# PauloMigAlmeida/MidoriDB

Hardware: AMD Instinct MI355X
Metric: joined rows/sec, 2x10^8-row INT64 INNER JOIN+GROUP BY, 1/2/4/8 MI355X (higher is better)
Workload: dtype int64

## Files before the change

### midoridb_amd/csrc/mdb_dev_leaf_wide.hip

```cpp
#include "mdb_dev_join_internal.h"

__device__ static inline uint4 lw_load_nt(const void *p)
{
	typedef unsigned int u4_nt __attribute__((ext_vector_type(4)));
	const u4_nt v = __builtin_nontemporal_load(reinterpret_cast<const u4_nt *>(p));
	return make_uint4(v.x, v.y, v.z, v.w);
}


template <bool HAS_R, bool R16 = false >
__global__ __launch_bounds__(LW_THREADS) void k_leaf_wide(gc_args a, uint32_t rem, uint32_t shift, uint32_t nsub)
{
	extern __shared__ __attribute__((aligned(16))) uint32_t lw_lds[];
	__shared__ unsigned long long s_red[LW_THREADS / 64];
	__shared__ uint32_t s_scan[32];
	__shared__ uint32_t s_base;
	const uint32_t T = 1u << rem, mask = T - 1u, leaf = blockIdx.x;
	uint32_t *const s_first = lw_lds;
	uint32_t *const s_cl = lw_lds + T;
	uint32_t *const s_cr = lw_lds + T + T / 2;
	for (uint32_t s = threadIdx.x; s < T; s += LW_THREADS)
		s_first[s] = 0xFFFFFFFFu;
	for (uint32_t s = threadIdx.x; s < (HAS_R ? T : T / 2); s += LW_THREADS)
		s_cl[s] = 0u;
// ... 653 lines not shown
			if (a.keyed_cbits && (cmax >> a.keyed_cbits))
				mdb_raise(a.status, 256u);
			if (!a.keyed_cbits && (cmax >> (32 - (a.kbits < 32 ? a.kbits : 31))))
				mdb_raise(a.status, 16u | (a.rec32 ? 512u : 0u));
		}
		const unsigned long long sums = ((unsigned long long)sum_cl << 32) | (NX ? 0u : sum_cr);
		const unsigned long long want = ((unsigned long long)adds << 32) | radds;
		unsigned long long diff = sums - want;
#pragma unroll
		for (int o = 32; o; o >>= 1)
			diff += __shfl_down(diff, o, MDB_WAVE);
		lw12_barrier();
		if (lane == 0)
			s_red[wave] = diff;
		lw12_barrier();
		diff = 0ull;
#pragma unroll
		for (int w = 0; w < LW_THREADS / 64; w++)
			diff += s_red[w];
		if (diff != 0ull || prod_bad) {
			bad = true;
			break;
		}
	}
	if (bad && threadIdx.x == 0)
		mdb_raise(a.status, 1024u);
	joined = lw_block_sum(joined, s_red);
	if (threadIdx.x == 0 && joined)
		atomicAdd(a.joined, joined);
	if (DN) {
		const unsigned long long cl_all = lw_block_sum((unsigned long long)cleared, s_red);
		if (threadIdx.x == 0 && cl_all)
			atomicAdd(&a.dn_cnt[0], (uint32_t)cl_all);
	}
#pragma unroll
	for (int o = 32; o; o >>= 1) {
		const uint32_t other = (uint32_t)__shfl_xor((int)last_first, o, MDB_WAVE);
		last_first = other > last_first ? other : last_first;
	}
	__syncthreads();
	if (lane == 0)
		s_red[wave] = last_first;
	__syncthreads();
	if (threadIdx.x == 0) {
		uint32_t m = 0;
#pragma unroll
		for (int w = 0; w < LW_THREADS / 64; w++)
			m = (uint32_t)s_red[w] > m ? (uint32_t)s_red[w] : m;
		if (m)
			atomicMax(a.status + 9, m);
	}
}

__global__ __launch_bounds__(LW_THREADS, 8 ) void k_leaf_wide4(gc_args a, uint32_t rem, uint32_t shift, uint32_t nsub)
{
	extern __shared__ __attribute__((aligned(16))) uint32_t lw_lds[];
	__shared__ unsigned long long s_red[LW_THREADS / 64];
	__shared__ uint32_t s_red32[LW_THREADS / 64];
	__shared__ uint32_t s_base;
	const uint32_t T = 1u << rem, mask = T - 1u, leaf = blockIdx.x, wave = threadIdx.x >> 6, lane = mdb_lane();
	uint32_t *const s_fc = lw_lds;
	uint32_t *const s_cl = lw_lds + T;
	for (uint32_t s = threadIdx.x; s < T; s += LW_THREADS)
		s_fc[s] = 0x07FFFFFFu;
	for (uint32_t s = threadIdx.x; s < T / 8; s += LW_THREADS)
		s_cl[s] = 0u;
	uint32_t *const s_rg = s_cl + (T / 8 < 16u ? 16u : T / 8);
	if (a.rg_rec)
		for (uint32_t r = threadIdx.x; r < a.rg_n; r += LW_THREADS)
			s_rg[r] = 0u;
	__syncthreads();
	uint32_t rows_r = 0;
	{
		const uint16_t *const hv_r16 = reinterpret_cast<const uint16_t *>(a.hv_r);
		for (uint32_t sub = 0; sub < nsub; sub++) {
			const uint32_t c0 = a.cnt_r[sub * a.nleaves + leaf], c = c0 < a.cap_r ? c0 : a.cap_r;
			const uint16_t *const src = hv_r16 + (size_t)(leaf * nsub + sub) * a.cap_r;
			rows_r += c;
			for (uint32_t j0 = 0; j0 < c; j0 += 8u * LW_THREADS * LW_UNROLL) {
				uint4 v[LW_UNROLL];
#pragma unroll
				for (int u = 0; u < LW_UNROLL; u++) {
					const uint32_t j = j0 + 8u * ((uint32_t)u * LW_THREADS + threadIdx.x);
					v[u] = make_uint4(0u, 0u, 0u, 0u);
					if (j < c)
						v[u] = lw_load_nt(src + j);
				}
#pragma unroll
				for (int u = 0; u < LW_UNROLL; u++) {
					const uint32_t j = j0 + 8u * ((uint32_t)u * LW_THREADS + threadIdx.x);
					const uint32_t w[4] = { v[u].x, v[u].y, v[u].z, v[u].w };
					if (j + 8u <= c) {
#pragma unroll
						for (int k = 0; k < 8; k++)
							atomicAdd(&s_fc[(w[k >> 1] >> (16 * (k & 1))) & mask], 1u << 27);
					} else {
#pragma unroll
						for (int k = 0; k < 8; k++)
							if (j + k < c)
								atomicAdd(&s_fc[(w[k >> 1] >> (16 * (k & 1))) & mask], 1u << 27);
					}
				}
			}
		}
	}
	__syncthreads();
	uint32_t adds = 0;
	for (uint32_t sub = 0; sub < nsub; sub++) {
		const uint32_t c0 = a.cnt_l[sub * a.nleaves + leaf], c = c0 < a.cap_l ? c0 : a.cap_l;
		const uint64_t *const src = a.hv_l + (size_t)(leaf * nsub + sub) * a.cap_l;
		for (uint32_t i0 = 0; i0 < c; i0 += 2u * LW_THREADS * LW_UNROLL) {
			ulonglong2 v[LW_UNROLL];
#pragma unroll
			for (int u = 0; u < LW_UNROLL; u++) {
				const uint32_t i = i0 + 2u * ((uint32_t)u * LW_THREADS + threadIdx.x);
				v[u] = make_ulonglong2(0ull, 0ull);
				if (i < c)
					v[u] = *reinterpret_cast<const ulonglong2 *>(src + i);
			}
#pragma unroll
			for (int u = 0; u < LW_UNROLL; u++) {
				const uint32_t i = i0 + 2u * ((uint32_t)u * LW_THREADS + threadIdx.x);
				const unsigned long long w[2] = { v[u].x, v[u].y };
#pragma unroll
				for (int k = 0; k < 2; k++)
					if (i + k < c) {
						const uint32_t idx = ((uint32_t)(w[k] >> 32) >> shift) & mask, fc = s_fc[idx];
						if (fc >> 27) {
							atomicMin(&s_fc[idx], (fc & 0xF8000000u) | (uint32_t)w[k]);
							atomicAdd(&s_cl[idx >> 3], 1u << ((idx & 7u) * 4u));
							adds++;
						}
					}
			}
		}
	}
	__syncthreads();
	const uint32_t per_wave = T / (LW_THREADS / 64), words_per_wave = per_wave / 8;
	uint32_t mine = 0, sum_cl = 0, sum_cr = 0;
	for (uint32_t wi = lane; wi < words_per_wave; wi += MDB_WAVE) {
		const uint32_t cw = s_cl[wave * words_per_wave + wi];
		mine += (uint32_t)__popc((cw | (cw >> 1) | (cw >> 2) | (cw >> 3)) & 0x11111111u);
		sum_cl += (((cw & 0x0F0F0F0Fu) + ((cw >> 4) & 0x0F0F0F0Fu)) * 0x01010101u) >> 24;
	}
	{
		uint32_t t = mine;
#pragma unroll
		for (int o = 32; o; o >>= 1)
			t += (uint32_t)__shfl_xor((int)t, o, MDB_WAVE);
		if (lane == 0)
			s_red32[wave] = t;
	}
	__syncthreads();
	if (threadIdx.x == 0) {
		uint32_t total = 0;
#pragma unroll
		for (int w = 0; w < LW_THREADS / 64; w++)
			total += s_red32[w];
		uint32_t nb = 0xFFFFFFFFu;
		if (total && a.rg_rec) {
			atomicAdd(a.rec_valid, total);
			nb = 0u;
		} else if (total) {
			nb = atomicAdd(a.rec_count, total);
			if (nb + total > a.rec_cap) {
				mdb_raise(a.status, 8u);
				nb = 0xFFFFFFFFu;
			} else {
				atomicAdd(a.rec_valid, total);
			}
		}
		s_base = nb;
	}
	__syncthreads();
	const uint32_t base = s_base;
	uint32_t run = 0;
	{
		uint32_t t = lane < wave ? s_red32[lane] : 0u;
#pragma unroll
		for (int o = 32; o; o >>= 1)
			t += (uint32_t)__shfl_xor((int)t, o, MDB_WAVE);
		run = base + t;
	}
	const uint32_t nib = (lane & 7u) * 4u, s_begin = wave * per_wave + lane;
	uint32_t cmax = 0, jsum = 0, last_first = 0, clmax = 0;
	if (a.rg_rec && base != 0xFFFFFFFFu) {
		for (uint32_t s0 = 0; s0 < per_wave; s0 += MDB_WAVE) {
// ... 148 lines not shown
```

### midoridb_amd/csrc/mdb_dev_common.h

```cpp
#ifndef MDB_DEV_COMMON_H
#define MDB_DEV_COMMON_H

#include <hip/hip_runtime.h>
#include <stdint.h>
#include <stdio.h>
#include <string.h>
#include <vector>
#include <string>
#include <unordered_map>
#include "mdb_dev.h"

#define MDB_WAVE 64

struct mdb_prof_rec {
	int name_id;
	hipEvent_t start, stop;
};

struct mdb_col_memo {
	const void *nh_kl, *nh_kr;
	uint64_t nh_nl, nh_nr;
	int nh_result;
	int64_t nh_base;
	uint32_t nh_kbits;
// ... 94 lines not shown
	std::vector<std::vector<const void *>> prof_kernels;
	std::vector<mdb_prof_rec> prof_recs;
	std::vector<std::pair<hipEvent_t, hipEvent_t>> prof_pool;
	size_t prof_pool_used;
};

int mdb_set_err(mdb_dev_ctx *ctx, int code, const char *fmt, ...);
extern "C" int mdb_knob_set(const char *name);
extern "C" int mdb_knob_off(const char *name);
extern "C" long long mdb_knob_int(const char *name, long long dflt);
extern "C" int mdb_knob_str(const char *name, char *buf, size_t cap);

struct mdb_plan_scope {
	mdb_dev_ctx *c;
	explicit mdb_plan_scope(mdb_dev_ctx *ctx) : c(ctx)
	{
		if (c && c->pl_depth++ == 0)
			memset(&c->plan, 0, sizeof(c->plan));
	}
	~mdb_plan_scope()
	{
		if (c && --c->pl_depth == 0) {
			c->ct_calls++;
			c->ct_retries += c->plan.retries;
			c->ct_samples += c->plan.samples;
		}
	}
};

static inline void mdb_explain_sampled(mdb_dev_ctx *ctx)
{
	if (ctx->explain_as_sample) {
		ctx->plan.from_stats = 0;
		ctx->plan.samples = 1;
	}
}

void mdb_memo_switch(mdb_dev_ctx *ctx, const void *kl, uint64_t nl, const void *kr, uint64_t nr);

#define MDB_HIP(ctx, call)                                                                         \
	do {                                                                                       \
		hipError_t e__ = (call);                                                           \
		if (e__ != hipSuccess)                                                             \
			return mdb_set_err((ctx), -MIDORIDB_INTERNAL, "%s failed: %s (%s:%d)", #call, \
					   hipGetErrorString(e__), __FILE__, __LINE__);            \
	} while (0)

int mdb_cached_alloc(mdb_dev_ctx *ctx, size_t bytes, void **dptr);
int mdb_cached_free(mdb_dev_ctx *ctx, void *dptr);

int mdb_arena_begin(mdb_dev_ctx *ctx, size_t total_bytes);
void *mdb_arena_take(mdb_dev_ctx *ctx, size_t bytes);
#define MDB_ZERO_BLK_OFF 128u
#define MDB_ZERO_BLK_SLOT 4096u
#define MDB_ZERO_BLK_WORDS (2u * MDB_ZERO_BLK_SLOT + 2048u)
static inline size_t mdb_align_up(size_t x) { return (x + 255) & ~(size_t)255; }

int mdb_aux_begin(mdb_dev_ctx *ctx, hipStream_t *saved_main);
int mdb_aux_end(mdb_dev_ctx *ctx, hipStream_t saved_main);
int mdb_aux_join(mdb_dev_ctx *ctx);

void mdb_prof_begin(mdb_dev_ctx *ctx, const char *name, const void *kernel);
void mdb_prof_end(mdb_dev_ctx *ctx);

#define MDB_LAUNCH(ctx, name, kernel, grid, block, ...)                                            \
	do {                                                                                       \
		mdb_prof_begin((ctx), (name), (const void *)(kernel));                             \
		hipLaunchKernelGGL(kernel, dim3(grid), dim3(block), 0, (ctx)->stream, __VA_ARGS__); \
		mdb_prof_end((ctx));                                                               \
		hipError_t le__ = hipGetLastError();                                               \
		if (le__ != hipSuccess)                                                            \
			return mdb_set_err((ctx), -MIDORIDB_INTERNAL, "launch %s failed: %s", (name), \
					   hipGetErrorString(le__));                               \
	} while (0)

#define MDB_LAUNCH_LDS(ctx, name, kernel, grid, block, lds_bytes, ...)                             \
	do {                                                                                       \
		mdb_prof_begin((ctx), (name), (const void *)(kernel));                             \
		hipLaunchKernelGGL(kernel, dim3(grid), dim3(block), (lds_bytes), (ctx)->stream, __VA_ARGS__); \
		mdb_prof_end((ctx));                                                               \
		hipError_t le__ = hipGetLastError();                                               \
		if (le__ != hipSuccess)                                                            \
			return mdb_set_err((ctx), -MIDORIDB_INTERNAL, "launch %s failed: %s", (name), \
					   hipGetErrorString(le__));                               \
	} while (0)

#ifdef __HIPCC__

__host__ __device__ static inline uint64_t mdb_fmix64(uint64_t k)
{
	k ^= k >> 33;
	k *= 0xff51afd7ed558ccdULL;
	k ^= k >> 33;
	k *= 0xc4ceb9fe1a85ec53ULL;
	k ^= k >> 33;
	return k;
}

__host__ __device__ static inline uint32_t mdb_fmix32(uint32_t h)
{
	h ^= h >> 16;
	h *= 0x85EBCA6Bu;
	h ^= h >> 13;
	h *= 0xC2B2AE35u;
	h ^= h >> 16;
	return h;
// ... 78 lines not shown
```

### midoridb_amd/csrc/mdb_dev_partition.hip

```cpp
#include <stdlib.h>
#include <type_traits>
#include "mdb_dev_internal.h"

#define PART_THREADS 512
#define PART_WAVES (PART_THREADS / MDB_WAVE)
#define PART_ITEMS (MDB_TILE / PART_THREADS)
#define PART_WAVE_SPAN (MDB_TILE / PART_WAVES)
#define PART_MAX_R (1u << MDB_MAX_RADIX_BITS)
#define PART_FEW_DIGITS 4u
#define PART_INVALID 0xFFFFFFFFu

struct mdb_level_args {
	const int64_t *keys;
	const uint64_t *nullbits;
	uint64_t n;
	const uint64_t *hv_in;
	const uint32_t *rid_in;
	const mdb_tile_desc *tiles;
	uint64_t *hv_out;
	uint32_t *rid_out;
	uint32_t *hist;
	uint32_t ntiles;
	uint32_t R;
	uint32_t shift;
	uint32_t mbits;
	uint32_t mode;
	uint32_t inverse_out;
	uint32_t *cursor;
	uint32_t cap;
	uint32_t skip_zero;
	uint32_t nsub;
	uint32_t *status;
	uint32_t narrow;
	int64_t narrow_base;
	uint32_t narrow_kbits;
	uint32_t keys32;
	const uint32_t *filter;
	uint32_t filter_words, filter_shift;
	uint32_t *minmax_out;
	uint32_t *minmax_final;
	const uint32_t *range_in;
	unsigned long long *minmax64_out;
	const long long *range64_in;
	const uint64_t *pay_in[2];
	uint64_t *pay_out[2];
	uint32_t npay;
	uint32_t keep_on;
	int64_t keep_lo, keep_hi;
	uint32_t own_on;
	int64_t own_lo, own_hi;
	uint32_t out16_shift;
	uint32_t fold64;
};

template <bool CF = false, bool RIDW = false>
// ... 1064 lines not shown
		a.keep_on = (flt && l == 0 && flt->keep_on) ? 1u : 0u;
		a.keep_lo = flt ? flt->keep_lo : 0;
		a.keep_hi = flt ? flt->keep_hi : 0;
		a.minmax_out = (flt && l == 0 && flt->minmax_out) ? flt->minmax_tiles : NULL;
		a.minmax_final = a.minmax_out ? flt->minmax_out : NULL;
		a.range_in = (flt && l == 0) ? flt->range_in : NULL;
		a.minmax64_out = (flt && l == 0 && flt->minmax64_out) ? flt->minmax64_tiles : NULL;
		a.range64_in = (flt && l == 0) ? flt->range64_in : NULL;
		a.filter = (flt && l == 1) ? flt->bits : NULL;
		a.filter_words = flt ? flt->words : 0u;
		a.filter_shift = flt ? flt->shift : 0u;
		if (a.mode == MDB_DIGIT_RADIX) {
			const int b = l == 0 ? bits1 : bits2;
			a.shift = (uint32_t)((w32 ? 32 : 64) - used_bits - b);
			a.mbits = (uint32_t)b;
		} else {
			uint32_t mb = 1;
			while ((1u << mb) < R)
				mb++;
			a.shift = 0;
			a.mbits = mb;
		}

		if (fast0 && l == 0) {
			const bool cursor_ext = !dry && flt && flt->cursor0_ext && nreg0 <= flt->cursor0_ext_words;
			uint32_t *cursor0 = cursor_ext ? flt->cursor0_ext : (uint32_t *)cv.take((size_t)nreg0 * 4);
			uint32_t *reg_nt = (uint32_t *)cv.take(((size_t)nreg0 + 1) * 4);
			const uint32_t next_tiles = (uint32_t)(n / MDB_TILE) + nreg0 + 1;
			mdb_tile_desc *next_desc = stop0 ? NULL : (mdb_tile_desc *)cv.take((size_t)next_tiles * sizeof(mdb_tile_desc));
			if (cv.failed)
				return -MIDORIDB_INTERNAL;
			if (!dry) {
				const bool cf = a.narrow && narrow_kbits && !(flags & PART_F_KEYS32) && mode == MDB_DIGIT_RADIX && !raw_hv && !want_rid;
				a.cursor = cursor0;
				a.cap = cap0;
				a.nsub = PART_NSUB;
				a.status = ctx->d_status;
				if (!cursor_ext)
					MDB_HIP(ctx, hipMemsetAsync(cursor0, 0, (size_t)nreg0 * 4, ctx->stream));
				const long long t2min = mdb_knob_int("MDB_TILE2_MIN", 0);
				const bool t2 = n >= (t2min > 0 ? (uint64_t)t2min : (1ull << 25)) &&
						!mdb_knob_off("MDB_TILE2");
				const uint32_t ntiles2 = (uint32_t)((n + (uint64_t)PART_TMUL * MDB_TILE - 1) / ((uint64_t)PART_TMUL * MDB_TILE));
				if (raw_hv && fold32 && t2) {
					a.ntiles = ntiles2;
					MDB_LAUNCH(ctx, "sort_scatter_l0_w32", (k_part_scatter<pf_word_raw_w32_t2>), grid8(ntiles2), PART_THREADS, a);
				} else if (raw_hv && fold32) {
					MDB_LAUNCH(ctx, "sort_scatter_l0_w32", (k_part_scatter<pf_word_raw_w32>), grid8(ntiles), PART_THREADS, a);
				} else if (raw_hv) {
					MDB_LAUNCH(ctx, "sort_scatter_l0", (k_part_scatter<pf_word_raw>), grid8(ntiles), PART_THREADS, a);
				} else if (w32) {
					if (out16) {
						a.out16_shift = 32u - narrow_kbits;
						if (cf && t2) {
							a.ntiles = ntiles2;
							MDB_LAUNCH(ctx, "part_scatter_l0_w32", (k_part_scatter<pf_key_w32_out16_cf_t2>),
								   grid8(ntiles2), PART_THREADS, a);
						} else if (cf) {
							MDB_LAUNCH(ctx, "part_scatter_l0_w32", (k_part_scatter<pf_key_w32_out16_cf>),
								   grid8(ntiles), PART_THREADS, a);
						} else {
							MDB_LAUNCH(ctx, "part_scatter_l0_w32", (k_part_scatter<pf_key_w32_out16>),
								   grid8(ntiles), PART_THREADS, a);
						}
					} else if (cf) {
						MDB_LAUNCH(ctx, "part_scatter_l0_w32", (k_part_scatter<pf_key_w32_cf>),
							   grid8(ntiles), PART_THREADS, a);
					} else {
						MDB_LAUNCH(ctx, "part_scatter_l0_w32", (k_part_scatter<pf_key_w32>), grid8(ntiles), PART_THREADS, a);
					}
					if (a.minmax_out)
						MDB_LAUNCH(ctx, "part_minmax", k_part_minmax_reduce, MM_GROUPS, MM_THREADS, (const uint32_t *)a.minmax_out, a.ntiles, flt->minmax_out);
				} else if (npay) {
					if (!cf || a.narrow != 1u)
						return mdb_set_err(ctx, -MIDORIDB_INTERNAL, "payload cells travel with the compact narrow form's hash | row id words only");
					a.npay = (uint32_t)npay;
					for (int c = 0; c < npay; c++) {
						a.pay_in[c] = reinterpret_cast<const uint64_t *>(flt->pay_in[c]);
						a.pay_out[c] = pay_buf[c];
					}
					MDB_LAUNCH(ctx, "part_scatter_l0_pay", (k_part_scatter<pf_key_cf_pay>), grid8(ntiles), PART_THREADS, a);
				} else if (want_rid && a.range64_in) {
					MDB_LAUNCH(ctx, "part_scatter_l0_rid_pruned", (k_part_scatter<pf_key_rid_r64>), grid8(ntiles), PART_THREADS, a);
				} else if (want_rid) {
					MDB_LAUNCH(ctx, "part_scatter_l0_rid", (k_part_scatter<pf_key_rid>), grid8(ntiles), PART_THREADS, a);
				} else if (a.minmax64_out) {
					MDB_LAUNCH(ctx, "part_scatter_l0", (k_part_scatter<pf_key_mm64>), grid8(ntiles), PART_THREADS, a);
					MDB_LAUNCH(ctx, "part_minmax", k_part_minmax64_reduce, 1, 1024, (const unsigned long long *)a.minmax64_out, ntiles,
						   flt->minmax64_out);
				} else if (a.range_in && cf && t2) {
					a.ntiles = ntiles2;
					MDB_LAUNCH(ctx, "part_scatter_l0_pruned", (k_part_scatter<pf_key_cf_t2>), grid8(ntiles2), PART_THREADS, a);
				} else if (a.range_in && cf) {
					MDB_LAUNCH(ctx, "part_scatter_l0_pruned", (k_part_scatter<pf_key_cf>),
						   grid8(ntiles), PART_THREADS, a);
				} else if (a.range_in) {
					MDB_LAUNCH(ctx, "part_scatter_l0_pruned", (k_part_scatter<pf_key>), grid8(ntiles), PART_THREADS, a);
				} else if (cf && t2) {
					a.ntiles = ntiles2;
					MDB_LAUNCH(ctx, "part_scatter_l0", (k_part_scatter<pf_key_cf_t2>), grid8(ntiles2), PART_THREADS, a);
				} else if (cf) {
					MDB_LAUNCH(ctx, "part_scatter_l0", (k_part_scatter<pf_key_cf>), grid8(ntiles),
						   PART_THREADS, a);
				} else {
					MDB_LAUNCH(ctx, "part_scatter_l0", (k_part_scatter<pf_key>), grid8(ntiles), PART_THREADS, a);
				}
				if (!stop0) {
// ... 372 lines not shown
```

Measured before the change: 178.7 billion.

## Flatten leaf_wide4 sub-region loops into a double-buffered cursor loader

Replaces the per-sub-region nested loops in k_leaf_wide4 with one flattened iteration space. A per-block prefix scan of the sub-region counts is kept in LDS, and a wave-uniform cursor maps chunk indices to addresses. Loads are double-buffered (two register batches of depth 3), so global loads for the next batch are issued while LDS atomics run on the current one. This also removes tail inefficiency on small sub-regions. In exchange it adds a cap of 8 sub-regions with an error raise, extra cursor arithmetic and register pressure, and it drops the barrier between the right and left phases.

```diff
diff --git a/midoridb_amd/csrc/mdb_dev_leaf_wide.hip b/midoridb_amd/csrc/mdb_dev_leaf_wide.hip
--- a/midoridb_amd/csrc/mdb_dev_leaf_wide.hip
+++ b/midoridb_amd/csrc/mdb_dev_leaf_wide.hip
@@ -729,6 +729,52 @@
 	}
 }
 
+#define LW_NSUB 8u
+#define LW4_DEPTH 3
+
+struct lw_cursor {
+	uint32_t j, c0, c1, cnt;
+};
+
+__device__ static inline lw_cursor lw_cursor_begin(const uint32_t *seg)
+{
+	lw_cursor at;
+	at.j = 0u;
+	at.c0 = 0u;
+	at.c1 = (uint32_t)__builtin_amdgcn_readfirstlane((int)seg[LW_NSUB]);
+	at.cnt = (uint32_t)__builtin_amdgcn_readfirstlane((int)seg[0]);
+	return at;
+}
+
+template <uint32_t PER, bool NT, typename W>
+__device__ static inline uint32_t lw_chunk_load(const W *tbl, uint32_t cap, const uint32_t *seg, uint32_t total, lw_cursor &at, uint32_t q, uint4 &v)
+{
+	const uint32_t last = total - 1u, q0 = (uint32_t)__builtin_amdgcn_readfirstlane((int)q);
+	const uint32_t q_lo = q0 < last ? q0 : last, q_hi = q0 + (MDB_WAVE - 1u) < last ? q0 + (MDB_WAVE - 1u) : last, qc = q < last ? q : last;
+	while (q_lo >= at.c1 && at.j + 1u < LW_NSUB) {
+		at.j++;
+		at.c0 = at.c1;
+		at.c1 = (uint32_t)__builtin_amdgcn_readfirstlane((int)seg[LW_NSUB + at.j]);
+		at.cnt = (uint32_t)__builtin_amdgcn_readfirstlane((int)seg[at.j]);
+	}
+	uint32_t first = at.c0, words = at.cnt, skip = 0u;
+	if (q_hi >= at.c1) {
+		uint32_t jj = at.j, c1 = at.c1;
+		while (qc >= c1 && jj + 1u < LW_NSUB) {
+			first = c1;
+			jj++;
+			c1 = seg[LW_NSUB + jj];
+		}
+		words = seg[jj];
+		skip = (jj - at.j) * cap;
+	}
+	const uint32_t word = (qc - first) * PER;
+	const char *const src = reinterpret_cast<const char *>(tbl + (size_t)at.j * cap) + (uint32_t)((skip + word) * (uint32_t)sizeof(W));
+	v = NT ? lw_load_nt(src) : *reinterpret_cast<const uint4 *>(src);
+	const uint32_t nv = words - word < PER ? words - word : PER;
+	return q < total ? nv : 0u;
+}
+
 __global__ __launch_bounds__(LW_THREADS, 8 ) void k_leaf_wide4(gc_args a, uint32_t rem, uint32_t shift, uint32_t nsub)
 {
 	extern __shared__ __attribute__((aligned(16))) uint32_t lw_lds[];
@@ -738,6 +784,16 @@
 	const uint32_t T = 1u << rem, mask = T - 1u, leaf = blockIdx.x, wave = threadIdx.x >> 6, lane = mdb_lane();
 	uint32_t *const s_fc = lw_lds;
 	uint32_t *const s_cl = lw_lds + T;
+	if (nsub > LW_NSUB || (((uint64_t)(a.cap_l > a.cap_r ? a.cap_l : a.cap_r) * (8u * LW_NSUB)) >> 32)) {
+		if (threadIdx.x == 0)
+			mdb_raise(a.status, 4096u);
+		return;
+	}
+	uint32_t *const s_seg = reinterpret_cast<uint32_t *>(s_red);
+	static_assert(4u * LW_NSUB * sizeof(uint32_t) <= sizeof(s_red), "the counts of a digit's sub-regions do not fit s_red");
+	uint32_t seg_cnt = 0;
+	if (threadIdx.x < 2u * LW_NSUB && (threadIdx.x & (LW_NSUB - 1u)) < nsub)
+		seg_cnt = (threadIdx.x < LW_NSUB ? a.cnt_r : a.cnt_l)[(threadIdx.x & (LW_NSUB - 1u)) * a.nleaves + leaf];
 	for (uint32_t s = threadIdx.x; s < T; s += LW_THREADS)
 		s_fc[s] = 0x07FFFFFFu;
 	for (uint32_t s = threadIdx.x; s < T / 8; s += LW_THREADS)
@@ -746,70 +802,101 @@
 	if (a.rg_rec)
 		for (uint32_t r = threadIdx.x; r < a.rg_n; r += LW_THREADS)
 			s_rg[r] = 0u;
+	{
+		const uint32_t seg_cap = threadIdx.x < LW_NSUB ? a.cap_r : a.cap_l;
+		seg_cnt = seg_cnt < seg_cap ? seg_cnt : seg_cap;
+		uint32_t run = threadIdx.x < LW_NSUB ? (seg_cnt + 7u) >> 3 : (seg_cnt + 1u) >> 1;
+#pragma unroll
+		for (uint32_t o = 1; o < LW_NSUB; o <<= 1) {
+			const uint32_t before = (uint32_t)__shfl_up((int)run, o, (int)LW_NSUB);
+			if ((threadIdx.x & (LW_NSUB - 1u)) >= o)
+				run += before;
+		}
+		if (threadIdx.x < 2u * LW_NSUB) {
+			const uint32_t at = (threadIdx.x / LW_NSUB) * 2u * LW_NSUB + (threadIdx.x & (LW_NSUB - 1u));
+			s_seg[at] = seg_cnt;
+			s_seg[at + LW_NSUB] = run;
+		}
+	}
 	__syncthreads();
 	uint32_t rows_r = 0;
-	{
-		const uint16_t *const hv_r16 = reinterpret_cast<const uint16_t *>(a.hv_r);
-		for (uint32_t sub = 0; sub < nsub; sub++) {
-			const uint32_t c0 = a.cnt_r[sub * a.nleaves + leaf], c = c0 < a.cap_r ? c0 : a.cap_r;
-			const uint16_t *const src = hv_r16 + (size_t)(leaf * nsub + sub) * a.cap_r;
-			rows_r += c;
-			for (uint32_t j0 = 0; j0 < c; j0 += 8u * LW_THREADS * LW_UNROLL) {
-				uint4 v[LW_UNROLL];
-#pragma unroll
-				for (int u = 0; u < LW_UNROLL; u++) {
-					const uint32_t j = j0 + 8u * ((uint32_t)u * LW_THREADS + threadIdx.x);
-					v[u] = make_uint4(0u, 0u, 0u, 0u);
-					if (j < c)
-						v[u] = lw_load_nt(src + j);
-				}
-#pragma unroll
-				for (int u = 0; u < LW_UNROLL; u++) {
-					const uint32_t j = j0 + 8u * ((uint32_t)u * LW_THREADS + threadIdx.x);
-					const uint32_t w[4] = { v[u].x, v[u].y, v[u].z, v[u].w };
-					if (j + 8u <= c) {
-#pragma unroll
-						for (int k = 0; k < 8; k++)
+#pragma unroll
+	for (int j = 0; j < (int)LW_NSUB; j++)
+		rows_r += s_seg[j];
+	const uint32_t total_r = (uint32_t)__builtin_amdgcn_readfirstlane((int)s_seg[2u * LW_NSUB - 1u]);
+	const uint32_t total_l = (uint32_t)__builtin_amdgcn_readfirstlane((int)s_seg[4u * LW_NSUB - 1u]);
+	if (total_r) {
+		const uint16_t *const hv_r16 = reinterpret_cast<const uint16_t *>(a.hv_r) + (size_t)leaf * nsub * a.cap_r;
+		lw_cursor at = lw_cursor_begin(s_seg);
+		uint4 va[LW4_DEPTH], vb[LW4_DEPTH];
+		auto issue_r = [&](uint32_t batch, uint4(&v)[LW4_DEPTH]) -> uint32_t {
+			uint32_t nvs = 0;
+#pragma unroll
+			for (int u = 0; u < LW4_DEPTH; u++)
+				nvs |= lw_chunk_load<8u, true>(hv_r16, a.cap_r, s_seg, total_r, at, (batch * LW4_DEPTH + (uint32_t)u) * LW_THREADS + threadIdx.x, v[u]) << (4 * u);
+			return nvs;
+		};
+		auto count_r = [&](const uint4(&v)[LW4_DEPTH], uint32_t nvs) {
+#pragma unroll
+			for (int u = 0; u < LW4_DEPTH; u++) {
+				const uint32_t w[4] = { v[u].x, v[u].y, v[u].z, v[u].w }, nv = (nvs >> (4 * u)) & 15u;
+				if (nv == 8u) {
+#pragma unroll
+					for (int k = 0; k < 8; k++)
+						atomicAdd(&s_fc[(w[k >> 1] >> (16 * (k & 1))) & mask], 1u << 27);
+				} else {
+#pragma unroll
+					for (int k = 0; k < 8; k++)
+						if ((uint32_t)k < nv)
 							atomicAdd(&s_fc[(w[k >> 1] >> (16 * (k & 1))) & mask], 1u << 27);
-					} else {
-#pragma unroll
-						for (int k = 0; k < 8; k++)
-							if (j + k < c)
-								atomicAdd(&s_fc[(w[k >> 1] >> (16 * (k & 1))) & mask], 1u << 27);
-					}
-				}
-			}
-		}
-	}
-	__syncthreads();
+				}
+			}
+		};
+		const uint32_t nbat = (total_r + LW4_DEPTH * LW_THREADS - 1u) / (LW4_DEPTH * LW_THREADS);
+		uint32_t na = issue_r(0u, va), nb;
+		for (uint32_t b = 0; b < nbat; b += 2u) {
+			nb = issue_r(b + 1u, vb);
+			count_r(va, na);
+			na = issue_r(b + 2u, va);
+			count_r(vb, nb);
+		}
+	}
 	uint32_t adds = 0;
-	for (uint32_t sub = 0; sub < nsub; sub++) {
-		const uint32_t c0 = a.cnt_l[sub * a.nleaves + leaf], c = c0 < a.cap_l ? c0 : a.cap_l;
-		const uint64_t *const src = a.hv_l + (size_t)(leaf * nsub + sub) * a.cap_l;
-		for (uint32_t i0 = 0; i0 < c; i0 += 2u * LW_THREADS * LW_UNROLL) {
-			ulonglong2 v[LW_UNROLL];
-#pragma unroll
-			for (int u = 0; u < LW_UNROLL; u++) {
-				const uint32_t i = i0 + 2u * ((uint32_t)u * LW_THREADS + threadIdx.x);
-				v[u] = make_ulonglong2(0ull, 0ull);
-				if (i < c)
-					v[u] = *reinterpret_cast<const ulonglong2 *>(src + i);
-			}
-#pragma unroll
-			for (int u = 0; u < LW_UNROLL; u++) {
-				const uint32_t i = i0 + 2u * ((uint32_t)u * LW_THREADS + threadIdx.x);
-				const unsigned long long w[2] = { v[u].x, v[u].y };
+	if (total_l) {
+		const uint64_t *const hv_l = a.hv_l + (size_t)leaf * nsub * a.cap_l;
+		lw_cursor at = lw_cursor_begin(s_seg + 2u * LW_NSUB);
+		uint4 va[LW4_DEPTH], vb[LW4_DEPTH];
+		auto issue_l = [&](uint32_t batch, uint4(&v)[LW4_DEPTH]) -> uint32_t {
+			uint32_t nvs = 0;
+#pragma unroll
+			for (int u = 0; u < LW4_DEPTH; u++)
+				nvs |= lw_chunk_load<2u, false>(hv_l, a.cap_l, s_seg + 2u * LW_NSUB, total_l, at, (batch * LW4_DEPTH + (uint32_t)u) * LW_THREADS + threadIdx.x, v[u]) << (4 * u);
+			return nvs;
+		};
+		auto count_l = [&](const uint4(&v)[LW4_DEPTH], uint32_t nvs) {
+#pragma unroll
+			for (int u = 0; u < LW4_DEPTH; u++) {
+				const uint32_t w[4] = { v[u].x, v[u].y, v[u].z, v[u].w }, nv = (nvs >> (4 * u)) & 15u;
 #pragma unroll
 				for (int k = 0; k < 2; k++)
-					if (i + k < c) {
-						const uint32_t idx = ((uint32_t)(w[k] >> 32) >> shift) & mask, fc = s_fc[idx];
+					if ((uint32_t)k < nv) {
+						const uint32_t idx = (w[2 * k + 1] >> shift) & mask, fc = s_fc[idx];
 						if (fc >> 27) {
-							atomicMin(&s_fc[idx], (fc & 0xF8000000u) | (uint32_t)w[k]);
+							atomicMin(&s_fc[idx], (fc & 0xF8000000u) | w[2 * k]);
 							atomicAdd(&s_cl[idx >> 3], 1u << ((idx & 7u) * 4u));
 							adds++;
 						}
 					}
 			}
+		};
+		const uint32_t nbat = (total_l + LW4_DEPTH * LW_THREADS - 1u) / (LW4_DEPTH * LW_THREADS);
+		uint32_t na = issue_l(0u, va), nb = issue_l(1u, vb);
+		lw12_barrier();
+		for (uint32_t b = 0; b < nbat; b += 2u) {
+			count_l(va, na);
+			na = issue_l(b + 2u, va);
+			count_l(vb, nb);
+			nb = issue_l(b + 3u, vb);
 		}
 	}
 	__syncthreads();
diff --git a/profiles/leaf_wide4_loader/cmp_dumps.py b/profiles/leaf_wide4_loader/cmp_dumps.py
--- /dev/null
+++ b/profiles/leaf_wide4_loader/cmp_dumps.py
@@ -0,0 +1,17 @@
+import glob
+import os
+import sys
+
+import numpy as np
+
+a, b = sys.argv[1], sys.argv[2]
+fa = sorted(os.path.basename(f) for f in glob.glob(a + "/*.npy"))
+fb = sorted(os.path.basename(f) for f in glob.glob(b + "/*.npy"))
+assert fa and fa == fb, (fa, fb)
+for f in fa:
+    x, y = np.load(os.path.join(a, f)), np.load(os.path.join(b, f))
+    same = x.shape == y.shape and np.array_equal(x, y)
+    print(f, x.shape, "identical" if same else "DIFFERENT")
+    assert same
+    os.remove(os.path.join(a, f))
+    os.remove(os.path.join(b, f))
diff --git a/profiles/leaf_wide4_loader/kstats.py b/profiles/leaf_wide4_loader/kstats.py
--- /dev/null
+++ b/profiles/leaf_wide4_loader/kstats.py
@@ -0,0 +1,16 @@
+import csv
+import glob
+import statistics
+import sys
+
+d, tag = sys.argv[1], sys.argv[2]
+rows = {}
+for f in glob.glob(d + "/**/*kernel_trace.csv", recursive=True):
+    with open(f) as fh:
+        for r in csv.DictReader(fh):
+            rows.setdefault(r["Kernel_Name"], []).append((int(r["End_Timestamp"]) - int(r["Start_Timestamp"])) / 1000.0)
+for k, v in sorted(rows.items(), key=lambda kv: -sum(kv[1])):
+    if sum(v) < 50 and "leaf_wide4" not in k:
+        continue
+    sd = statistics.pstdev(v) if len(v) > 1 else 0.0
+    print(f"{tag} {k.split('(')[0][:60]:60s} n={len(v):3d} avg_us={statistics.mean(v):8.1f} sd_us={sd:6.1f} min_us={min(v):8.1f}")
```

After: 176.6 billion. 0.988x the previous value.

## Add persistent streaming 512-way level-0 scatter kernel with fused min/max reduction

Applied to the files above, without the earlier changes.

Adds a persistent-grid scatter kernel for the 32-bit-key, 16-bit-output level-0 partition. Each workgroup streams over a contiguous row range, using a register ring of nontemporal prefetched loads. It overlaps counting of the next tile with the scattered stores of the previous tile, which are staged in LDS. The separate min/max reduction launch is folded into the kernel using a last-block ticket. This costs more LDS and register pressure, plus a specialised path with tighter eligibility conditions.

```diff
diff --git a/midoridb_amd/csrc/mdb_dev_common.h b/midoridb_amd/csrc/mdb_dev_common.h
--- a/midoridb_amd/csrc/mdb_dev_common.h
+++ b/midoridb_amd/csrc/mdb_dev_common.h
@@ -170,6 +170,7 @@
 int mdb_arena_begin(mdb_dev_ctx *ctx, size_t total_bytes);
 void *mdb_arena_take(mdb_dev_ctx *ctx, size_t bytes);
 #define MDB_ZERO_BLK_OFF 128u
+#define MDB_ST_TICKET 48u
 #define MDB_ZERO_BLK_SLOT 4096u
 #define MDB_ZERO_BLK_WORDS (2u * MDB_ZERO_BLK_SLOT + 2048u)
 static inline size_t mdb_align_up(size_t x) { return (x + 255) & ~(size_t)255; }
diff --git a/midoridb_amd/csrc/mdb_dev_partition.hip b/midoridb_amd/csrc/mdb_dev_partition.hip
--- a/midoridb_amd/csrc/mdb_dev_partition.hip
+++ b/midoridb_amd/csrc/mdb_dev_partition.hip
@@ -1,6 +1,7 @@
 #include <stdlib.h>
 #include <type_traits>
 #include "mdb_dev_internal.h"
+#include "mdb_dev_scatter512.h"
 
 #define PART_THREADS 512
 #define PART_WAVES (PART_THREADS / MDB_WAVE)
@@ -1171,7 +1172,39 @@
 				} else if (w32) {
 					if (out16) {
 						a.out16_shift = 32u - narrow_kbits;
-						if (cf && t2) {
+						const bool stream = cf && t2 && !a.range_in && !a.keep_on && !a.own_on && n >= 1 && n < (1ull << 31) && R <= S512_D &&
+								    (!a.minmax_out || a.minmax_final) && !mdb_knob_off("MDB_STREAM512");
+						if (stream) {
+							s512_args sa;
+							memset(&sa, 0, sizeof(sa));
+							sa.keys = reinterpret_cast<const long long *>(keys);
+							sa.nullbits = reinterpret_cast<const unsigned long long *>(nullbits);
+							sa.n = (uint32_t)n;
+							sa.key_lo = narrow_base;
+							sa.kbits = narrow_kbits;
+							sa.rem = narrow_kbits - (uint32_t)bits1;
+							sa.R = R;
+							sa.out = reinterpret_cast<uint16_t *>(a.hv_out);
+							sa.cursor = cursor0;
+							sa.cap = cap0;
+							sa.nsub = PART_NSUB;
+							sa.status = ctx->d_status;
+							const uint32_t s_tile = S512_THREADS * S512_RPT;
+							const uint32_t s_grid = s512_grid(keys, sa.n, s_tile, S512_WG_PER_CU * (uint32_t)ctx->num_cus, &sa.rows_per_wg);
+							sa.mm_wg = a.minmax_out;
+							sa.mm_ticket = ctx->d_status + MDB_ST_TICKET;
+							sa.mm_final = a.minmax_final;
+							const size_t lds = s512_stream_lds(s_tile);
+							if (sa.mm_wg && nullbits)
+								MDB_LAUNCH_LDS(ctx, "part_scatter_l0_w32", (k_scatter512_stream<S512_THREADS, S512_RPT, true, true>), s_grid, S512_THREADS, lds, sa);
+							else if (sa.mm_wg)
+								MDB_LAUNCH_LDS(ctx, "part_scatter_l0_w32", (k_scatter512_stream<S512_THREADS, S512_RPT, false, true>), s_grid, S512_THREADS, lds, sa);
+							else if (nullbits)
+								MDB_LAUNCH_LDS(ctx, "part_scatter_l0_w32", (k_scatter512_stream<S512_THREADS, S512_RPT, true, false>), s_grid, S512_THREADS, lds, sa);
+							else
+								MDB_LAUNCH_LDS(ctx, "part_scatter_l0_w32", (k_scatter512_stream<S512_THREADS, S512_RPT, false, false>), s_grid, S512_THREADS, lds, sa);
+							a.minmax_out = NULL;
+						} else if (cf && t2) {
 							a.ntiles = ntiles2;
 							MDB_LAUNCH(ctx, "part_scatter_l0_w32", (k_part_scatter<pf_key_w32_out16_cf_t2>),
 								   grid8(ntiles2), PART_THREADS, a);
diff --git a/midoridb_amd/csrc/mdb_dev_scatter512.h b/midoridb_amd/csrc/mdb_dev_scatter512.h
--- /dev/null
+++ b/midoridb_amd/csrc/mdb_dev_scatter512.h
@@ -0,0 +1,311 @@
+#ifndef MDB_DEV_SCATTER512_H
+#define MDB_DEV_SCATTER512_H
+
+#include "mdb_dev_scatter4096.h"
+
+#define S512_D 512u
+#define S512_THREADS 512
+#define S512_RPT 32
+#define S512_RING 8
+#define S512_WG_PER_CU 2u
+
+struct s512_args {
+	const long long *keys;
+	const unsigned long long *nullbits;
+	uint32_t n;
+	long long key_lo;
+	uint32_t kbits, rem;
+	uint32_t R;
+	uint16_t *out;
+	uint32_t *cursor;
+	uint32_t cap, nsub;
+	uint32_t *status;
+	uint32_t rows_per_wg;
+	uint32_t *mm_wg, *mm_ticket, *mm_final;
+};
+
+__device__ static inline uint32_t s512_mixk(uint32_t x, uint32_t s, uint32_t mask)
+{
+	x ^= x >> s;
+	x = (x * 0x85EBCA6Bu) & mask;
+	x ^= x >> s;
+	x = (x * 0xC2B2AE35u) & mask;
+	x ^= x >> s;
+	return x;
+}
+
+template <int THREADS, int RPT , bool NULLS = false, bool MM = true , int RING_ = S512_RING,
+	  int ABLATE = 0 >
+__global__ __launch_bounds__(THREADS, 4 ) void k_scatter512_stream(s512_args a)
+{
+	constexpr uint32_t TILE = THREADS * RPT, D = S512_D, NCHUNK = TILE / 64u, NPAIR = RPT / 2, RING = RING_;
+	constexpr uint32_t WB = 4;
+	static_assert(TILE <= 32768u && THREADS == (int)D && RPT % 4 == 0 && NPAIR % RING == 0 && (TILE / 32u) % 2u == 0, "tile shape");
+	extern __shared__ __attribute__((aligned(16))) uint32_t s512_lds[];
+	uint32_t *const s_cnt = s512_lds;
+	uint32_t *const s_delta = s_cnt + D + 64;
+	uint32_t *const s_chunk = s_delta + D;
+	uint32_t *const s_mark = s_chunk + NCHUNK;
+	uint32_t *const s_tmp = s_mark + TILE / 32u;
+	uint16_t *const s_stage = reinterpret_cast<uint16_t *>(s_tmp + 32);
+	__shared__ uint32_t s_any_bad, s_last;
+
+	const uint32_t lane = mdb_lane(), sub = blockIdx.x % a.nsub, R = a.R;
+	const uint32_t none = R << a.rem;
+	const uint32_t hmask = a.kbits >= 32u ? 0xFFFFFFFFu : ((1u << a.kbits) - 1u), hshift = (a.kbits + 1u) >> 1;
+	const uint64_t limit = (1ull << a.kbits) - 1ull;
+	const uint64_t le = mdb_lanemask_lt() | (1ull << lane);
+	const uint32_t lead = (uint32_t)(reinterpret_cast<uintptr_t>(a.keys) >> 3) & 1u;
+	const long long *const fkeys = a.keys - lead;
+	const uint32_t nf = a.n + lead;
+	for (uint32_t i = threadIdx.x; i < D + 64; i += THREADS)
+		s_cnt[i] = 0u;
+	if (threadIdx.x == 0)
+		s_any_bad = 0u;
+	uint32_t seen_min = 0xFFFFFFFFu, seen_max = 0u;
+
+	const uint32_t r_begin = blockIdx.x * a.rows_per_wg;
+	const uint32_t r_end = r_begin >= nf ? r_begin : (nf - r_begin > a.rows_per_wg ? r_begin + a.rows_per_wg : nf);
+
+	ulonglong2 pre[RING];
+	uint32_t hs[RPT];
+#define S512_REQUEST(P, t0, tlen, tid_)                                                                                  \
+	do {                                                                                                             \
+		if (ABLATE & 2) {                                                                                        \
+			const unsigned long long i_ = (t0) + 2u * ((uint32_t)(P) * THREADS + (tid_));                    \
+			pre[(P) % RING] = make_ulonglong2((unsigned long long)a.key_lo + ((i_ * 0x9E3779B1ull) & limit), \
+							  (unsigned long long)a.key_lo + (((i_ + 1u) * 0x9E3779B1ull) & limit)); \
+		} else {	 \
+			typedef unsigned long long ull2_nt_ __attribute__((ext_vector_type(2)));                         \
+			const uint32_t last_ = ((tlen) - 1u) & ~1u, e0_ = 2u * ((uint32_t)(P) * THREADS + (tid_));      \
+			const ull2_nt_ v_ = __builtin_nontemporal_load(reinterpret_cast<const ull2_nt_ *>(              \
+				reinterpret_cast<const char *>(fkeys + (t0)) + (size_t)(e0_ < last_ ? e0_ : last_) * 8u)); \
+			pre[(P) % RING] = make_ulonglong2(v_.x, v_.y);                                                   \
+		}                                                                                                        \
+	} while (0)
+#define S512_COUNT(r_, t0, tlen, tid_)                                                                                   \
+	do {                                                                                                             \
+		const uint32_t e_ = 2u * ((uint32_t)((r_) >> 1) * THREADS + (tid_)) + (uint32_t)((r_) & 1);             \
+		const unsigned long long kk_ = ((r_) & 1) ? pre[((r_) >> 1) % RING].y : pre[((r_) >> 1) % RING].x;      \
+		bool ok_ = e_ < (tlen) && (t0) + e_ >= lead;                                                             \
+		if (NULLS && ok_) {                                                                                      \
+			const uint32_t row_ = (t0) + e_ - lead;                                                          \
+			ok_ = !((a.nullbits[row_ >> 6] >> (row_ & 63u)) & 1ull);                                         \
+		}                                                                                                        \
+		const unsigned long long rel_ = kk_ - (unsigned long long)a.key_lo;                                      \
+		const bool take_ = ok_ && rel_ <= limit;                                                                 \
+		oow |= ok_ && !take_;                                                                                    \
+		if (MM) {                                                                                                \
+			seen_min = min(seen_min, take_ ? (uint32_t)rel_ : 0xFFFFFFFFu);                                  \
+			seen_max = max(seen_max, take_ ? (uint32_t)rel_ : 0u);                                           \
+		}                                                                                                        \
+		uint32_t h_ = s512_mixk((uint32_t)rel_, hshift, hmask);	 \
+		asm volatile("" : "+v"(h_));                                                                             \
+		h_ = take_ ? h_ : none;                                                                                  \
+		atomicAdd(&s_cnt[h_ >> a.rem], 1u);                                                                      \
+		hs[r_] = h_;                                                                                             \
+	} while (0)
+
+	uint32_t row0 = r_begin, staged_row0 = 0;
+	uint32_t len = (r_end - row0) < TILE ? (r_end - row0) : TILE, staged_total = 0u;
+	if (len) {
+		uint32_t tid = threadIdx.x;
+		asm volatile("" : "+v"(tid));
+#pragma unroll
+		for (int p = 0; p < (int)RING; p++)
+			S512_REQUEST(p, row0, len, tid);
+	}
+	shw_barrier();
+
+	for (;;) {
+		uint32_t tid = threadIdx.x;
+		asm volatile("" : "+v"(tid));
+		const uint32_t wave = tid >> 6;
+		const uint32_t nrow0 = row0 + len;
+		const uint32_t nlen = len ? ((r_end - nrow0) < TILE ? (r_end - nrow0) : TILE) : 0u;
+		const uint32_t prow0 = nlen ? nrow0 : row0;
+		const uint32_t plen = nlen ? nlen : len;
+		bool oow = false;
+
+		if (len) {
+#pragma unroll
+			for (int k = 0; k < RPT; k++) {
+				S512_COUNT(k, row0, len, tid);
+				if (k & 1)
+					__builtin_amdgcn_sched_barrier(0);
+				if ((k & 1) && (k >> 1) + (int)RING < (int)NPAIR)
+					S512_REQUEST((k >> 1) + (int)RING, row0, len, tid);
+				else if (k & 1)
+					S512_REQUEST((k >> 1) + (int)RING - (int)NPAIR, prow0, plen, tid);
+			}
+			if (oow)
+				mdb_raise(a.status, 128u);
+		}
+#pragma unroll
+		for (int k0 = 0; k0 < RPT; k0 += (int)WB) {
+			if ((uint32_t)k0 * THREADS < staged_total) {
+				uint64_t m[WB];
+				uint32_t ord[WB], g[WB];
+				uint16_t sv[WB];
+#pragma unroll
+				for (int u = 0; u < (int)WB; u++) {
+					const uint32_t c = (uint32_t)(k0 + u) * (THREADS / 64) + wave;
+					m[u] = *reinterpret_cast<const uint64_t *>(&s_mark[2u * c]);
+					ord[u] = s_chunk[c];
+					sv[u] = s_stage[(uint32_t)(k0 + u) * THREADS + tid];
+				}
+#pragma unroll
+				for (int u = 0; u < (int)WB; u++) {
+					ord[u] += (uint32_t)__popcll(m[u] & le) - 1u;
+					ord[u] = ord[u] < D ? ord[u] : D - 1u;
+					g[u] = s_delta[ord[u]];
+				}
+#pragma unroll
+				for (int u = 0; u < (int)WB; u++) {
+					const uint32_t i = (uint32_t)(k0 + u) * THREADS + tid;
+					const bool put = i < staged_total;
+					uint32_t gi = i + g[u];
+					if (ABLATE & 16)
+						gi = staged_row0 + i;
+					if (!(ABLATE & 1)) {
+						if (put)
+							a.out[gi] = sv[u];
+					} else if (put && sv[u] == (uint16_t)0xFFF1u && gi == 0xFFFFFFFFu) {
+						a.out[0] = sv[u];
+					}
+				}
+			}
+		}
+		shw_barrier();
+		if (!len)
+			break;
+
+		const uint32_t cnt = tid < R ? s_cnt[tid] : 0u;
+		for (uint32_t i = tid; i < TILE / 32u; i += THREADS)
+			s_mark[i] = 0u;
+		if (tid == 0)
+			s_chunk[0] = 0u;
+		uint32_t tot;
+		const uint32_t ex = shw_block_excl_scan(cnt + (cnt ? 65536u : 0u), s_tmp, THREADS / 64, &tot);
+		const uint32_t tile_total = (uint32_t)__builtin_amdgcn_readfirstlane((int)(tot & 0xFFFFu));
+		const uint32_t start = ex & 0xFFFFu, ord = ex >> 16;
+		uint32_t base = 0u;
+		if (cnt) {
+			base = atomicAdd(&a.cursor[sub * R + tid], cnt);
+			atomicOr(&s_mark[start >> 5], 1u << (start & 31u));
+			for (uint32_t c = (start >> 6) + 1u; (c << 6) <= start + cnt && c < NCHUNK; c++)
+				s_chunk[c] = ord + 1u;
+		}
+		if (tid < R)
+			s_cnt[tid] = start;
+		if (tid == 0)
+			s_cnt[R] = TILE;
+		shw_barrier();
+
+#pragma unroll
+		for (int r = 0; r < RPT; r++) {
+			uint32_t pos = atomicAdd(&s_cnt[hs[r] >> a.rem], 1u);
+			pos = pos < TILE ? pos : TILE;
+			s_stage[pos] = (uint16_t)hs[r];
+		}
+		if (cnt) {
+			if (base + cnt > a.cap) {
+				mdb_raise(a.status, 2u);
+				s_any_bad = 1u;
+			}
+			s_delta[ord] = (tid * a.nsub + sub) * a.cap + base - start;
+		}
+		shw_barrier();
+		s_cnt[tid] = 0u;
+		if (tid == 0)
+			s_cnt[D] = 0u;
+		staged_total = __builtin_amdgcn_readfirstlane((int)s_any_bad) ? 0u : tile_total;
+		staged_row0 = row0;
+		row0 = nrow0;
+		len = nlen;
+		shw_barrier();
+		if (tid == 0)
+			s_any_bad = 0u;
+	}
+#undef S512_REQUEST
+#undef S512_COUNT
+
+	if (MM) {
+		const uint32_t wave = threadIdx.x >> 6;
+#pragma unroll
+		for (int o = MDB_WAVE / 2; o > 0; o >>= 1) {
+			seen_min = min(seen_min, (uint32_t)__shfl_xor((int)seen_min, o, MDB_WAVE));
+			seen_max = max(seen_max, (uint32_t)__shfl_xor((int)seen_max, o, MDB_WAVE));
+		}
+		if (lane == 0) {
+			s_tmp[2u * wave] = seen_min;
+			s_tmp[2u * wave + 1u] = seen_max;
+		}
+		__syncthreads();
+		if (threadIdx.x == 0) {
+			uint32_t mn = 0xFFFFFFFFu, mx = 0u;
+#pragma unroll
+			for (int w = 0; w < THREADS / 64; w++) {
+				mn = min(mn, s_tmp[2 * w]);
+				mx = max(mx, s_tmp[2 * w + 1]);
+			}
+			__hip_atomic_store(&a.mm_wg[2u * blockIdx.x], mn, __ATOMIC_RELAXED, __HIP_MEMORY_SCOPE_AGENT);
+			__hip_atomic_store(&a.mm_wg[2u * blockIdx.x + 1u], mx, __ATOMIC_RELAXED, __HIP_MEMORY_SCOPE_AGENT);
+			__threadfence();
+			s_last = atomicAdd(a.mm_ticket, 1u) == gridDim.x - 1u;
+		}
+		__syncthreads();
+		if (s_last) {
+			__threadfence();
+			uint32_t mn = 0xFFFFFFFFu, mx = 0u;
+			for (uint32_t b = threadIdx.x; b < gridDim.x; b += THREADS) {
+				mn = min(mn, __hip_atomic_load(&a.mm_wg[2u * b], __ATOMIC_RELAXED, __HIP_MEMORY_SCOPE_AGENT));
+				mx = max(mx, __hip_atomic_load(&a.mm_wg[2u * b + 1u], __ATOMIC_RELAXED, __HIP_MEMORY_SCOPE_AGENT));
+			}
+#pragma unroll
+			for (int o = MDB_WAVE / 2; o > 0; o >>= 1) {
+				mn = min(mn, (uint32_t)__shfl_xor((int)mn, o, MDB_WAVE));
+				mx = max(mx, (uint32_t)__shfl_xor((int)mx, o, MDB_WAVE));
+			}
+			if (lane == 0) {
+				s_tmp[2u * wave] = mn;
+				s_tmp[2u * wave + 1u] = mx;
+			}
+			__syncthreads();
+			if (threadIdx.x == 0) {
+				mn = 0xFFFFFFFFu;
+				mx = 0u;
+#pragma unroll
+				for (int w = 0; w < THREADS / 64; w++) {
+					mn = min(mn, s_tmp[2 * w]);
+					mx = max(mx, s_tmp[2 * w + 1]);
+				}
+				a.mm_final[0] = mn;
+				a.mm_final[1] = mx;
+				__hip_atomic_store(a.mm_ticket, 0u, __ATOMIC_RELAXED, __HIP_MEMORY_SCOPE_AGENT);
+			}
+		}
+	}
+}
+
+static inline size_t s512_stream_lds(uint32_t tile)
+{
+	return (size_t)4 * (S512_D + 64 + S512_D + tile / 64 + tile / 32 + 32) + 2 * ((size_t)tile + 64);
+}
+
+static inline uint32_t s512_grid(const void *keys, uint32_t n, uint32_t tile, uint32_t slots, uint32_t *rows_per_wg)
+{
+	const uint64_t nf = (uint64_t)n + ((reinterpret_cast<uintptr_t>(keys) >> 3) & 1u);
+	uint64_t grid = (nf + tile - 1) / tile;
+	if (grid > slots)
+		grid = slots;
+	if (grid < 1)
+		grid = 1;
+	uint64_t rpw = ((nf + grid - 1) / grid + 1) & ~1ull;
+	while (grid > 1 && (grid - 1) * rpw >= nf)
+		grid--;
+	*rows_per_wg = (uint32_t)rpw;
+	return (uint32_t)grid;
+}
+
+#endif
diff --git a/profiles/micro/scatter512_stream.hip b/profiles/micro/scatter512_stream.hip
--- /dev/null
+++ b/profiles/micro/scatter512_stream.hip
@@ -0,0 +1,226 @@
+#include "mdb_dev_partition.hip"
+#include <cstdlib>
+#include <vector>
+#include <algorithm>
+
+#define CK(x) do { hipError_t e_ = (x); if (e_ != hipSuccess) { printf("%s: %s (line %d)\n", #x, hipGetErrorString(e_), __LINE__); exit(1); } } while (0)
+#define NSUB 8u
+#define KBITS 23u
+#define DBITS 9u
+#define KEY_LO 1000ll
+#define MULT 0x9E3779B1ull
+
+__global__ void k_gen(long long *keys, uint32_t n, uint32_t nv)
+{
+	for (uint32_t i = blockIdx.x * blockDim.x + threadIdx.x; i < n; i += gridDim.x * blockDim.x)
+		keys[i] = KEY_LO + (long long)(((unsigned long long)(i % nv) * MULT) % nv);
+}
+
+__global__ void k_expect(const long long *keys, uint32_t n, uint32_t *expect)
+{
+	for (uint32_t i = blockIdx.x * blockDim.x + threadIdx.x; i < n; i += gridDim.x * blockDim.x)
+		atomicAdd(&expect[(uint32_t)(keys[i] - KEY_LO)], 1u);
+}
+
+__global__ void k_walk(const uint16_t *out, const uint32_t *cursor, uint32_t cap, uint32_t *got, unsigned long long *stats )
+{
+	const uint32_t D = 1u << DBITS, rem = KBITS - DBITS, r = blockIdx.x * blockDim.x + threadIdx.x;
+	if (r >= D * NSUB)
+		return;
+	const uint32_t d = r / NSUB, sub = r % NSUB;
+	uint32_t cnt = cursor[sub * D + d];
+	unsigned long long rows = 0, err = 0;
+	if (cnt > cap) {
+		err++;
+		cnt = cap;
+	}
+	const uint16_t *w = out + (size_t)r * cap;
+	for (uint32_t i = 0; i < cnt; i++) {
+		const uint32_t h = (d << rem) | (w[i] & ((1u << rem) - 1u));
+		if ((h & 0xFFFFu) != w[i]) {
+			err++;
+			continue;
+		}
+		atomicAdd(&got[mdb_unmixk(h, KBITS)], 1u);
+		rows++;
+	}
+	atomicAdd(&stats[0], rows);
+	atomicAdd(&stats[1], err);
+}
+
+__global__ void k_compare(const uint32_t *expect, const uint32_t *got, uint32_t nvals, unsigned long long *stats)
+{
+	for (uint32_t i = blockIdx.x * blockDim.x + threadIdx.x; i < nvals; i += gridDim.x * blockDim.x)
+		if (expect[i] != got[i])
+			atomicAdd(&stats[1], 1ull);
+}
+
+struct bufs {
+	long long *keys;
+	unsigned long long *nullbits;
+	uint16_t *out;
+	uint32_t *cursor, *status, *expect, *got, *mm;
+	unsigned long long *stats;
+	uint32_t n, nv, cap;
+};
+
+static void check(bufs &b, bool range)
+{
+	uint32_t st[64];
+	unsigned long long h[2];
+	CK(hipMemset(b.got, 0, (size_t)4 << KBITS));
+	CK(hipMemset(b.stats, 0, 16));
+	hipLaunchKernelGGL(k_walk, dim3((NSUB << DBITS) / 64), dim3(64), 0, 0, b.out, b.cursor, b.cap, b.got, b.stats);
+	hipLaunchKernelGGL(k_compare, dim3(1024), dim3(256), 0, 0, b.expect, b.got, 1u << KBITS, b.stats);
+	CK(hipDeviceSynchronize());
+	CK(hipMemcpy(h, b.stats, 16, hipMemcpyDeviceToHost));
+	CK(hipMemcpy(st, b.status, 256, hipMemcpyDeviceToHost));
+	const bool range_ok = !range || (st[16] == 0u && st[17] == b.nv - 1u && st[MDB_ST_TICKET] == 0u);
+	printf("   check: rows %llu / %u, errors %llu, status %u, range [%u, %u] -> %s", h[0], b.n, h[1], st[0], st[16], st[17],
+	       (h[0] == b.n && h[1] == 0 && st[0] == 0 && range_ok) ? "OK" : "WRONG");
+}
+
+static double report(const char *name, std::vector<float> &ms, bufs &b, bool chk, bool range)
+{
+	std::sort(ms.begin(), ms.end());
+	const double med = ms[ms.size() / 2];
+	printf("%-52s min %.4f med %.4f max %.4f ms   own I/O %.2f TB/s", name, ms[0], med, ms.back(), 10.0 * b.n / med * 1e-9);
+	if (chk)
+		check(b, range);
+	printf("\n");
+	fflush(stdout);
+	return med;
+}
+
+static double run_old(const char *name, bufs &b, int reps, bool chk, bool reduce)
+{
+	mdb_level_args a;
+	memset(&a, 0, sizeof(a));
+	a.keys = reinterpret_cast<const int64_t *>(b.keys);
+	a.n = b.n;
+	a.hv_out = reinterpret_cast<uint64_t *>(b.out);
+	a.ntiles = (uint32_t)(((uint64_t)b.n + (uint64_t)PART_TMUL * MDB_TILE - 1) / ((uint64_t)PART_TMUL * MDB_TILE));
+	a.R = 1u << DBITS;
+	a.shift = 32u - DBITS;
+	a.mbits = DBITS;
+	a.mode = MDB_DIGIT_RADIX;
+	a.narrow = 2u;
+	a.narrow_base = KEY_LO;
+	a.narrow_kbits = KBITS;
+	a.out16_shift = 32u - KBITS;
+	a.cursor = b.cursor;
+	a.cap = b.cap;
+	a.nsub = NSUB;
+	a.status = b.status;
+	a.minmax_out = b.mm;
+	a.minmax_final = b.status + 16;
+	hipEvent_t e0, e1;
+	CK(hipEventCreate(&e0));
+	CK(hipEventCreate(&e1));
+	std::vector<float> ms(reps);
+	for (int r = -1; r < reps; r++) {
+		CK(hipMemsetAsync(b.cursor, 0, (NSUB << DBITS) * 4, 0));
+		CK(hipMemsetAsync(b.status, 0, 256, 0));
+		CK(hipEventRecord(e0, 0));
+		hipLaunchKernelGGL((k_part_scatter<pf_key_w32_out16_cf_t2>), dim3(grid8(a.ntiles)), dim3(PART_THREADS), 0, 0, a);
+		if (reduce)
+			hipLaunchKernelGGL(k_part_minmax_reduce, dim3(MM_GROUPS), dim3(MM_THREADS), 0, 0, (const uint32_t *)a.minmax_out, a.ntiles, a.minmax_final);
+		CK(hipEventRecord(e1, 0));
+		CK(hipEventSynchronize(e1));
+		CK(hipGetLastError());
+		if (r >= 0)
+			CK(hipEventElapsedTime(&ms[r], e0, e1));
+	}
+	return report(name, ms, b, chk, reduce);
+}
+
+template <typename K>
+static double run_new(const char *name, K kernel, uint32_t tile, bool nulls, bool mm, bufs &b, int reps, bool chk, int cus)
+{
+	s512_args a;
+	memset(&a, 0, sizeof(a));
+	a.keys = b.keys;
+	a.nullbits = nulls ? b.nullbits : NULL;
+	a.n = b.n;
+	a.key_lo = KEY_LO;
+	a.kbits = KBITS;
+	a.rem = KBITS - DBITS;
+	a.R = 1u << DBITS;
+	a.out = b.out;
+	a.cursor = b.cursor;
+	a.cap = b.cap;
+	a.nsub = NSUB;
+	a.status = b.status;
+	a.mm_wg = b.mm;
+	a.mm_ticket = b.status + MDB_ST_TICKET;
+	a.mm_final = b.status + 16;
+	const uint32_t grid = s512_grid(b.keys, b.n, tile, S512_WG_PER_CU * (uint32_t)cus, &a.rows_per_wg);
+	const size_t lds = s512_stream_lds(tile);
+	CK(hipFuncSetAttribute(reinterpret_cast<const void *>(kernel), hipFuncAttributeMaxDynamicSharedMemorySize, (int)lds));
+	hipEvent_t e0, e1;
+	CK(hipEventCreate(&e0));
+	CK(hipEventCreate(&e1));
+	std::vector<float> ms(reps);
+	for (int r = -1; r < reps; r++) {
+		CK(hipMemsetAsync(b.cursor, 0, (NSUB << DBITS) * 4, 0));
+		CK(hipMemsetAsync(b.status, 0, 256, 0));
+		CK(hipEventRecord(e0, 0));
+		hipLaunchKernelGGL(kernel, dim3(grid), dim3(S512_THREADS), lds, 0, a);
+		CK(hipEventRecord(e1, 0));
+		CK(hipEventSynchronize(e1));
+		CK(hipGetLastError());
+		if (r >= 0)
+			CK(hipEventElapsedTime(&ms[r], e0, e1));
+	}
+	return report(name, ms, b, chk, mm);
+}
+
+int main(int argc, char **argv)
+{
+	const uint32_t n = argc > 1 ? (uint32_t)strtoull(argv[1], NULL, 10) : 100000000u;
+	const int reps = argc > 2 ? atoi(argv[2]) : 9;
+	hipDeviceProp_t prop;
+	CK(hipGetDeviceProperties(&prop, 0));
+	const int cus = prop.multiProcessorCount;
+	bufs b;
+	b.n = n;
+	b.nv = n / 16u ? n / 16u : 1u;
+	if (b.nv > (1u << KBITS) || n >= (1u << 31)) {
+		printf("rows: at most 16 x 2^%u\n", KBITS);
+		return 1;
+	}
+	const uint64_t avg = ((uint64_t)n + (NSUB << DBITS) - 1) / (NSUB << DBITS);
+	b.cap = (uint32_t)((avg * 5 / 4 + 1024 + 63) & ~63ull);
+	CK(hipMalloc(&b.keys, (size_t)n * 8 + 64));
+	CK(hipMalloc(&b.nullbits, ((size_t)n + 63) / 64 * 8 + 64));
+	CK(hipMemset(b.nullbits, 0, ((size_t)n + 63) / 64 * 8 + 64));
+	CK(hipMalloc(&b.out, (size_t)(NSUB << DBITS) * b.cap * 2 + 4096));
+	CK(hipMalloc(&b.cursor, (NSUB << DBITS) * 4));
+	CK(hipMalloc(&b.status, 256));
+	CK(hipMalloc(&b.expect, (size_t)4 << KBITS));
+	CK(hipMalloc(&b.got, (size_t)4 << KBITS));
+	CK(hipMalloc(&b.mm, mdb_part_minmax_words(n) * 4));
+	CK(hipMalloc(&b.stats, 128));
+	CK(hipMemset(b.expect, 0, (size_t)4 << KBITS));
+	hipLaunchKernelGGL(k_gen, dim3(cus * 8), dim3(256), 0, 0, b.keys, n, b.nv);
+	hipLaunchKernelGGL(k_expect, dim3(cus * 8), dim3(256), 0, 0, b.keys, n, b.expect);
+	CK(hipDeviceSynchronize());
+	printf("%u rows, %u values, %d CUs, region capacity %u words, %d reps\n", n, b.nv, cus, b.cap, reps);
+	for (int round = 0; round < 2; round++) {
+		const bool chk = round == 0;
+		run_old("old  k_part_scatter<..._t2> + part_minmax", b, reps, chk, true);
+		run_old("old  k_part_scatter<..._t2> alone", b, reps, chk, false);
+		run_new("new  k_scatter512_stream<512,32> ring 8", k_scatter512_stream<512, 32, false, true, 8>, 16384, false, true, b, reps, chk, cus);
+		run_new("new  <512,32> ring 4", k_scatter512_stream<512, 32, false, true, 4>, 16384, false, true, b, reps, chk, cus);
+		run_new("new  <512,32> ring 16", k_scatter512_stream<512, 32, false, true, 16>, 16384, false, true, b, reps, chk, cus);
+		run_new("new  <512,48> ring 8 (24 576-row tiles)", k_scatter512_stream<512, 48, false, true, 8>, 24576, false, true, b, reps, chk, cus);
+		run_new("new  <512,64> ring 8 (32 768-row tiles)", k_scatter512_stream<512, 64, false, true, 8>, 32768, false, true, b, reps, chk, cus);
+		run_new("new  <512,32> ring 8, NULL bits", k_scatter512_stream<512, 32, true, true, 8>, 16384, true, true, b, reps, chk, cus);
+		run_new("new  <512,32> ring 8, no key range", k_scatter512_stream<512, 32, false, false, 8>, 16384, false, false, b, reps, chk, cus);
+	}
+	run_new("new  <512,32> ring 8, stores off", k_scatter512_stream<512, 32, false, true, 8, 1>, 16384, false, true, b, reps, false, cus);
+	run_new("new  <512,32> ring 8, loads off", k_scatter512_stream<512, 32, false, true, 8, 2>, 16384, false, true, b, reps, false, cus);
+	run_new("new  <512,32> ring 8, loads and stores off", k_scatter512_stream<512, 32, false, true, 8, 3>, 16384, false, true, b, reps, false, cus);
+	run_new("new  <512,32> ring 8, stores linear (whole lines)", k_scatter512_stream<512, 32, false, true, 8, 16>, 16384, false, true, b, reps, false, cus);
+	return 0;
+}
```

Result: slower. 178.1 billion before, 163.4 billion after (-8.2%).
